# lia2790/walking-controllers

Hardware: AMD Instinct MI355X
Metric: QP solves/sec (whole node), iCub IK-QP + DCM-MPC batch at 1/2/4/8 MI355X (higher is better)
Workload: dtype f64

## Files before the change

walking-controllers_amd/csrc/ik4.hip:

```cpp
#include "ik4_device.h"

namespace {

template <bool TICK, int JSRC, bool LOG = false, bool EXT = false>
__global__ __launch_bounds__(64, WCQP_IK4_WAVES)
void ik4_kernel(const IkDeviceParams* __restrict__ prm, int batch,
                const double* __restrict__ JL, const double* __restrict__ JR,
                const double* __restrict__ JN, const double* __restrict__ JC,
                const double* qpos, const double* __restrict__ state,
                double* __restrict__ dq_out, int* __restrict__ status_out,
                unsigned* __restrict__ alo_out, unsigned* __restrict__ aup_out,
                double* __restrict__ ferr_out, int* __restrict__ iters_out, const wcqp_tick::TickDev* __restrict__ tdp, int phase, int n_inner, int skip_last_mpc)
{
    __shared__ __attribute__((aligned(16))) double smem[4][PER_INST];
    if constexpr (TICK) {
        __shared__ __attribute__((aligned(16))) double kmodel[JSRC == 2 ? wcqp_tick::kKinTabSize : 2];
        __shared__ __attribute__((aligned(16))) double kgains[JSRC == 2 ? 4 * wcqp_tick::kGainsLdsStages : 2];
        ik4_tick_walk<JSRC, LOG, EXT, false>(prm, batch, JL, JR, JN, JC, qpos, state, dq_out, status_out, alo_out, aup_out, ferr_out, iters_out,
                                             tdp, phase, n_inner, skip_last_mpc, smem, kmodel, kgains);
    } else {
        ik4_body<TICK, JSRC>(prm, batch, JL, JR, JN, JC, qpos, state, dq_out, status_out, alo_out, aup_out, ferr_out, iters_out, wcqp_tick::TickDev{}, smem, xcd_group((int)blockIdx.x, (int)gridDim.x));
    }
}

// ... 21 lines not shown
                    unsigned* __restrict__ alo_out, unsigned* __restrict__ aup_out,
                    double* __restrict__ ferr_out, int* __restrict__ iters_out, int ik_blocks, MpcPairArgs m)
{
    __shared__ __attribute__((aligned(16))) double smem[4][PER_INST];
    const bool is_mpc = (int)blockIdx.x >= ik_blocks;
    const int blk = is_mpc ? (int)blockIdx.x - ik_blocks : xcd_group((int)blockIdx.x, ik_blocks);
    if (is_mpc) {
        static_assert(wcqp_mpc::kInstPerWave * WCQP_HULL_ROWS * 4 <= 4 * PER_INST, "the hull rows fit the IK's LDS");
        double (*s_hull)[WCQP_HULL_ROWS][4] = reinterpret_cast<double (*)[WCQP_HULL_ROWS][4]>(&smem[0][0]);
        const int lane = threadIdx.x;
        const int sub = lane / wcqp_mpc::kLanesPerInstance, t = lane % wcqp_mpc::kLanesPerInstance;
        const long inst_raw = (long)blk * wcqp_mpc::kInstPerWave + sub;
        const bool live = inst_raw < batch;
        const long inst = live ? inst_raw : (long)batch - 1;
        const double2* rp = reinterpret_cast<const double2*>(m.ref) + inst * m.ref_len;
        double ux, uy, margin;
        int st;
        unsigned mask;
        wcqp_mpc::mpc_row_solve(m.c, t, inst, m.x0, rp, m.ref_len, m.u_prev, m.hull_A, m.hull_b, m.hull_nc, inst, s_hull[sub], ux, uy, st, mask, margin);
        if (t == 0 && live) {
            reinterpret_cast<double2*>(m.u0)[inst] = make_double2(ux, uy);
            m.status[inst] = st;
            if (m.active) m.active[inst] = mask;
            if (m.margin) m.margin[inst] = margin;
        }
        return;
    }
    ik4_body<false>(prm, batch, JL, JR, JN, JC, qpos, state, dq_out, status_out, alo_out, aup_out, ferr_out, iters_out, wcqp_tick::TickDev{}, smem, blk);
}

template <bool WITH_MPC>
__device__ __forceinline__
void plan_walk(const IkDeviceParams* __restrict__ prm, int batch, const wcqp_qp_step* __restrict__ recs, int n_steps, int ways, int groups,
               const wcqp_mpc::MpcDeviceConsts& c, unsigned* queue, double (*smem)[PER_INST])
{
    const bool dynamic = ways == 0;
    unsigned z = threadIdx.x;
    __asm__ volatile("" : "+v"(z));
    z >>= 6;
    constexpr unsigned QS = wcqp_ik::kPlanQueueStride / 4u;
    const unsigned total = (unsigned)n_steps * (unsigned)groups;
    unsigned home = blockIdx.x % wcqp_ik::kPlanQueues;
    auto draw = [&]() -> unsigned {
#ifndef WCQP_PLAN_STEAL
#define WCQP_PLAN_STEAL (wcqp_ik::kPlanQueues - 1u)
#endif
        for (unsigned tried = 0; tried <= WCQP_PLAN_STEAL; ++tried) {
            unsigned k = 0;
            if (threadIdx.x == 0) k = __hip_atomic_fetch_add(queue + home * QS + z, 1u, __ATOMIC_RELAXED, __HIP_MEMORY_SCOPE_AGENT);
            const unsigned u = (unsigned)__builtin_amdgcn_readfirstlane((int)k) * wcqp_ik::kPlanQueues + home;
            if (u < total) return u;
            home = (home + 1u) % wcqp_ik::kPlanQueues;
        }
        return total;
    };
    int r = (int)blockIdx.x / groups, blk = (int)blockIdx.x % groups;
#ifndef WCQP_PLAN_NO_XCD_MAP
    if ((groups & 7) == 0) {
        const int n = groups >> 3, x = (int)blockIdx.x & 7, k = (int)blockIdx.x >> 3;
        r = k / n; blk = x * n + k % n;
    }
#endif
    if (dynamic) {
        const unsigned u = draw();
        r = u < total ? (int)(u % (unsigned)n_steps) : n_steps; blk = u < total ? (int)(u / (unsigned)n_steps) : 0;
    }
#pragma unroll 1
    while (r < n_steps) {
        __asm__ volatile("" ::: "memory");
        using wcqp::as_global;
        const wcqp_qp_step& s = recs[r];
        MpcPairArgs m{c, WITH_MPC ? as_global(s.x0) : nullptr, WITH_MPC ? as_global(s.ref) : nullptr, s.ref_len, WITH_MPC ? as_global(s.u_prev) : nullptr,
                      WITH_MPC ? as_global(s.hull_A) : nullptr, WITH_MPC ? as_global(s.hull_b) : nullptr, WITH_MPC ? as_global(s.hull_nc) : nullptr,
                      WITH_MPC ? as_global(s.u0) : nullptr, WITH_MPC ? as_global(s.mpc_status) : nullptr, WITH_MPC ? as_global(s.mpc_active) : nullptr,
                      WITH_MPC ? as_global(s.mpc_margin) : nullptr,
                      dynamic ? queue + home * QS + z : nullptr, 0u, WITH_MPC};
        ik4_body<false, 0, true>(prm, batch, as_global(s.J_left), as_global(s.J_right), as_global(s.J_neck), as_global(s.J_com), as_global(s.q), as_global(s.state),
                                 as_global(s.dq), as_global(s.ik_status), as_global(s.active_lower), as_global(s.active_upper),
                                 as_global(s.foot_err), as_global(s.iters), wcqp_tick::TickDev{}, smem, blk, 0, true, nullptr, nullptr, &m);
        wcqp::wave_lds_fence();
        if (dynamic) {
            unsigned u = (unsigned)__builtin_amdgcn_readfirstlane((int)m.ticket) * wcqp_ik::kPlanQueues + home;
            if (u >= total) { home = (home + 1u) % wcqp_ik::kPlanQueues; u = draw(); }
            r = u < total ? (int)(u % (unsigned)n_steps) : n_steps; blk = u < total ? (int)(u / (unsigned)n_steps) : 0;
        } else {
            r += ways;
        }
    }
    if (dynamic && threadIdx.x == 0) {
        __threadfence();
        if (atomicAdd(queue + wcqp_ik::kPlanQueues * QS, 1u) == gridDim.x - 1) {
            for (unsigned q = 0; q <= wcqp_ik::kPlanQueues; ++q) queue[q * QS] = 0u;
        }
    }
}

__global__ __launch_bounds__(64, WCQP_IK4_WAVES)
void qp_plan_kernel(const IkDeviceParams* __restrict__ prm, int batch, const wcqp_qp_step* __restrict__ recs, int n_steps, int ways, int groups,
                    wcqp_mpc::MpcDeviceConsts c, unsigned* queue)
{
    __shared__ __attribute__((aligned(16))) double smem[4][PER_INST];
    plan_walk<true>(prm, batch, recs, n_steps, ways, groups, c, queue, smem);
}
__global__ __launch_bounds__(64, WCQP_IK4_WAVES) WCQP_IK_PLAN_REGS
void ik_plan_kernel(const IkDeviceParams* __restrict__ prm, int batch, const wcqp_qp_step* __restrict__ recs, int n_steps, int ways, int groups,
                    wcqp_mpc::MpcDeviceConsts c, unsigned* queue)
{
    __shared__ __attribute__((aligned(16))) double smem[4][PER_INST];
    plan_walk<false>(prm, batch, recs, n_steps, ways, groups, c, queue, smem);
}

}

namespace wcqp_ik {

int ik4_plan_queue_grid(int batch, int n_steps) {
    int dev = 0, cus = 0;
    if (hipGetDevice(&dev) != hipSuccess || hipDeviceGetAttribute(&cus, hipDeviceAttributeMultiprocessorCount, dev) != hipSuccess || cus < 1) return -1;
    const long long total = (long long)((batch + 3) / 4) * n_steps, slots = (long long)cus * 4 * WCQP_IK4_WAVES;
    return (int)(total < slots ? total : slots);
}

int ik4_launch_plan(const IkDeviceParams* d_prm, int batch, const wcqp_qp_step* d_recs, int n_steps, int ways,
                    const wcqp_mpc::MpcDeviceConsts& c, hipStream_t stream, unsigned* d_queue, int queue_grid, bool ik_only) {
    if (!d_prm || !d_recs || batch < 1 || n_steps < 1 || ways < 0 || (ways == 0 && (!d_queue || queue_grid < 1))) return WCQP_E_INVALID;
    const int groups = (batch + 3) / 4;
    if ((long long)groups * n_steps >= (1ll << 31)) return WCQP_E_INVALID;
    const unsigned grid = ways == 0 ? (unsigned)queue_grid : (unsigned)(groups * ways);
    if (ik_only) hipLaunchKernelGGL(ik_plan_kernel, dim3(grid), dim3(64), 0, stream, d_prm, batch, d_recs, n_steps, ways, groups, c, d_queue);
    else hipLaunchKernelGGL(qp_plan_kernel, dim3(grid), dim3(64), 0, stream, d_prm, batch, d_recs, n_steps, ways, groups, c, d_queue);
    WCQP_HIP_TRY(hipGetLastError());
    return WCQP_OK;
}

int ik4_launch_pair(const IkDeviceParams* d_prm, int batch, const IkIo& io,
                    const wcqp_mpc::MpcDeviceConsts& c, const double* x0, const double* ref, int ref_len, const double* u_prev,
                    const double* hull_A, const double* hull_b, const int* hull_nc,
                    double* u0, int* mstatus, unsigned* mactive, double* mmargin, hipStream_t stream) {
    const int ik_blocks = (batch + 3) / 4;
    const int mpc_blocks = (batch + wcqp_mpc::kInstPerWave - 1) / wcqp_mpc::kInstPerWave;
    MpcPairArgs m{c, x0, ref, ref_len, u_prev, hull_A, hull_b, hull_nc, u0, mstatus, mactive, mmargin};
    hipLaunchKernelGGL(qp_pair_kernel, dim3((unsigned)(ik_blocks + mpc_blocks)), dim3(64), 0, stream, d_prm, batch,
// ... 58 lines not shown
```

walking-controllers_amd/csrc/ik4_device.h:

```cpp
#pragma once
#include <cmath>
#include <limits>
#include <type_traits>
#include "ik_common.h"
#include "tick_device.h"
#include "kin_device.h"

namespace {

using namespace wcqp_ik;

typedef double v4d __attribute__((ext_vector_type(4)));

constexpr int NR = 12;
constexpr int NROWS_IN = 18;
constexpr int KMAX = kDof - 9;
constexpr int LDC = 14;

constexpr int OFF_ST = 0;
constexpr int OFF_BV = 112;
constexpr int OFF_DB = 130;
constexpr int OFF_CT = 0;
constexpr int OFF_PB = 0;
constexpr int A_SIZE = 340;
constexpr int OFF_COL = A_SIZE;
constexpr int OFF_YV = A_SIZE + 32;
constexpr int OFF_DV = A_SIZE + 48;
constexpr int OFF_YPV = A_SIZE;
constexpr int OFF_RV = A_SIZE + 16;
constexpr int OFF_CV = A_SIZE + 32;
constexpr int OFF_ROWB = A_SIZE + 48;
constexpr int PER_INST = 440;
constexpr int K_FS = 14, K_TW = 0, K_FRB = 322, K_FR = 358;
constexpr int K_MS = 394, K_MH = 410;
// ... 29 lines not shown
#elif defined(WCQP_IK_STAMPS)
#define WCQP_STAMP(k) do { unsigned long long t__; asm volatile("s_memtime %0\n\ts_waitcnt lgkmcnt(0)" : "=s"(t__) :: "memory"); \
                           if (lane == __ffsll((long long)__ballot(true)) - 1) reinterpret_cast<unsigned long long*>(ferr_out)[(size_t)blockIdx.x * 16 + (k)] = t__; } while (0)
#else
#define WCQP_STAMP(k) do { } while (0)
#endif
#ifndef WCQP_KSTAMP
#define WCQP_KSTAMP(k) do { } while (0)
#endif

__device__ __forceinline__ void swap32(double& a, double& b) {
    const auto l = __builtin_amdgcn_permlane32_swap((unsigned)__double2loint(a), (unsigned)__double2loint(b), false, false);
    const auto h = __builtin_amdgcn_permlane32_swap((unsigned)__double2hiint(a), (unsigned)__double2hiint(b), false, false);
    a = __hiloint2double((int)h[0], (int)l[0]); b = __hiloint2double((int)h[1], (int)l[1]);
}
__device__ __forceinline__ void swap16(double& a, double& b) {
    const auto l = __builtin_amdgcn_permlane16_swap((unsigned)__double2loint(a), (unsigned)__double2loint(b), false, false);
    const auto h = __builtin_amdgcn_permlane16_swap((unsigned)__double2hiint(a), (unsigned)__double2hiint(b), false, false);
    a = __hiloint2double((int)h[0], (int)l[0]); b = __hiloint2double((int)h[1], (int)l[1]);
}

using wcqp_kin::st2;
using wcqp_kin::ld2;

struct MpcPairArgs {
    wcqp_mpc::MpcDeviceConsts c;
    const double* x0; const double* ref; int ref_len; const double* u_prev;
    const double* hull_A; const double* hull_b; const int* hull_nc;
    double* u0; int* status; unsigned* active; double* margin;
    unsigned* ticket_from = nullptr; unsigned ticket = 0;
    bool has_mpc = true;
};

template <bool TICK, int JSRC = 0, bool PAIR = false, bool LOG = false, bool EXT = false, bool REACT = false, bool GS = false, bool PL = false>
__device__ __forceinline__
void ik4_body(const IkDeviceParams* __restrict__ prm, int batch,
                const double* __restrict__ JL, const double* __restrict__ JR,
                const double* __restrict__ JN, const double* __restrict__ JC,
                const double* qpos, const double* __restrict__ state,
                double* __restrict__ dq_out, int* __restrict__ status_out,
                unsigned* __restrict__ alo_out, unsigned* __restrict__ aup_out,
                double* __restrict__ ferr_out, int* __restrict__ iters_out, const wcqp_tick::TickDev& td, double (*smem)[PER_INST], int blk,
                const int tick_now = 0, const bool do_mpc = true, const double* kmodel = nullptr, const double* gr_lds = nullptr,
                MpcPairArgs* pm = nullptr, double* carry = nullptr, int* gait = nullptr, const unsigned long long* noise_base = nullptr)
{
    static_assert(!(TICK && PAIR), "the tick kernel carries its own MPC chain");
    static_assert(TICK || !REACT, "the reactive controller is a tick form");
    static_assert(TICK || !GS, "gain scheduling is a tick form");
    static_assert(!PL || (TICK && JSRC == 2 && !LOG), "planned / streamed trajectories: the fused-kinematics tick without logger rows");
    constexpr bool ST = PL && EXT;
    constexpr bool COMPACT = JSRC == 1;
    constexpr bool KINF = JSRC == 2;
    int lane_id = threadIdx.x;
    if constexpr (TICK || PAIR) __asm__ volatile("" : "+v"(lane_id));
    const int lane = lane_id;
    const int grp = lane >> 4;
    const int j = lane & 15;
    const long inst_raw = (long)blk * 4 + grp;
    const bool live = inst_raw < batch;
    const long inst = live ? inst_raw : (long)batch - 1;
    using wcqp::at32;
    const unsigned iu = (unsigned)inst, j8 = (unsigned)j * 8u;
    double* S = smem[grp];
    double* st = S + OFF_ST;
    const double inf = std::numeric_limits<double>::infinity();
    const bool var1 = j < kDof - 16;
    const bool rhs1 = j == kDof - 16;
    const bool base1 = j >= 8 && j < 14;
    const int col1 = j + 16;

    unsigned prev_lo = 0u, prev_up = 0u;
    bool stopped = false;
    auto load_previous_set = [&]() {
        if (td.hot_start && alo_out && aup_out) { prev_lo = *at32(alo_out, iu * 4u); prev_up = *at32(aup_out, iu * 4u); }
        stopped = wcqp_tick::tick_robot_stopped(td, (int)inst);
        if (stopped) { prev_lo = 0u; prev_up = 0u; }
    };
    if constexpr (TICK && JSRC != 2) load_previous_set();

    WCQP_STAMP(0);
    const int v0i = 6 + j, v1i = var1 ? 22 + j : 0;
    double sd0, sd1, isd0, isd1, kq0, kq1, qreg0, qreg1;
    auto load_lane_constants = [&]() {
        sd0 = prm->sd[j]; sd1 = prm->sd[col1]; isd0 = prm->isd[j]; isd1 = prm->isd[col1];
        kq0 = prm->kq[v0i]; kq1 = prm->kq[v1i]; qreg0 = prm->qreg[v0i]; qreg1 = prm->qreg[v1i];
    };
    if constexpr (!KINF) load_lane_constants();
    double a0[NROWS_IN], a1[NROWS_IN];
    double q0, q1;
    double qm0, qm1;
    bool osqp_form;
    double k_pos_foot, k_att_foot, k_pos_com, kap;
    int fast_ok;
    wcqp_tick::TickMpcRegs mreg;
    double2 p_xs = make_double2(0.0, 0.0), p_up = make_double2(0.0, 0.0);
    if constexpr (PAIR) {
        if (pm->has_mpc) {
        wcqp_mpc::mpc_window_loads(pm->c, j, reinterpret_cast<const double2*>(pm->ref), iu * (unsigned)pm->ref_len, pm->ref_len, mreg.L);
        if (j == 0) { p_xs = *at32(reinterpret_cast<const double2*>(pm->x0), iu * 16u); p_up = *at32(reinterpret_cast<const double2*>(pm->u_prev), iu * 16u); }
        mreg.nc = *at32(pm->hull_nc, iu * 4u);
        mreg.ha = make_double2(0.0, 0.0); mreg.hb = 0.0;
        if (j < WCQP_HULL_ROWS) {
            mreg.ha = *at32(reinterpret_cast<const double2*>(pm->hull_A), (iu * WCQP_HULL_ROWS + (unsigned)j) * 16u);
            mreg.hb = *at32(pm->hull_b, iu * (WCQP_HULL_ROWS * 8u) + j8);
        }
        }
    }
    if constexpr (TICK && !REACT) { if (do_mpc) wcqp_tick::tick_mpc_issue<KINF>(td, j, inst, tick_now + 1, mreg); else mreg.phase0 = td.phase0[inst]; }
    double2 cr0[5], cr1[5], cdv[5];
    int ckind0 = 0, ckind1 = 0;
    double m_ux = 0.0, m_uy = 0.0;
    double2 m_r0 = make_double2(0.0, 0.0);
    double2 m_rd = make_double2(0.0, 0.0);
    if constexpr (TICK && REACT) { if (do_mpc) wcqp_tick::tick_react_issue(td, j, inst, tick_now + 1, mreg, m_r0, m_rd); else mreg.phase0 = td.phase0[inst]; }
    wcqp_tick::ZmpRegs zreg{};
    double m_s = 0.0;
    auto gsd = [&]() -> const wcqp_tick::TickDevGS& { return static_cast<const wcqp_tick::TickDevGS&>(td); };
    auto pld = [&]() -> const wcqp_tick::TickDevPL& { return static_cast<const wcqp_tick::TickDevPL&>(td); };
    double m_pf = 0.0;
    if constexpr (PL) { if (do_mpc) m_pf = wcqp_tick::plan_flags_issue<ST>(pld(), j, inst, tick_now + 1); }
    if constexpr (TICK && GS) {
        if (do_mpc) {
            wcqp_tick::zmp_state_issue(gsd(), inst, zreg);
            if constexpr (!REACT) m_rd = wcqp_tick::zmp_vel_issue(td, inst, tick_now + 1);
        }
    }
    {
        const unsigned so = iu * (unsigned)(kStateLen * 8);
        const double* sp = at32(state, so + j8);
        const double* sp5 = at32(state, so + 640u + (j < kStateLen - 80 ? j8 : 0u));
// ... 149 lines not shown
                }
                if (!REACT && j < 8) { const double* mh = S + K_MH + j * 3; mreg.ha.x = mh[0]; mreg.ha.y = mh[1]; mreg.hb = mh[2]; }
            }
        } else if constexpr (COMPACT) {
            const double* jb = td.jcomp + inst * td.cstride;
            const int off0 = wcqp_tick::compact_offset(td.cmaskL, td.cmaskR, td.cmaskN, j, ckind0);
            const int off1 = wcqp_tick::compact_offset(td.cmaskL, td.cmaskR, td.cmaskN, var1 ? col1 : 0, ckind1);
#pragma unroll
            for (int m = 0; m < 5; ++m) { cr0[m] = ld2(jb + off0 + 2 * m); cr1[m] = ld2(jb + off1 + 2 * m); }
#pragma unroll
            for (int m = 0; m < 5; ++m) cdv[m] = ld2(jb + td.coff_d + 2 * m);
        } else {
        const int fc0 = 6 + j;
        const int fc1 = var1 ? 22 + j : (base1 ? j - 8 : 0);
        const unsigned o6 = iu * (unsigned)(6 * kNV * 8), o3 = iu * (unsigned)(3 * kNV * 8), c0b = (unsigned)fc0 * 8u, c1b = (unsigned)fc1 * 8u;
        const double* jl0 = at32(JL, o6 + c0b), *jl1 = at32(JL, o6 + c1b);
        const double* jr0 = at32(JR, o6 + c0b), *jr1 = at32(JR, o6 + c1b);
        const double* jc0 = at32(JC, o3 + c0b), *jc1 = at32(JC, o3 + c1b);
        const double* jn0 = at32(JN, o3 + c0b), *jn1 = at32(JN, o3 + c1b);
#pragma unroll
        for (int r = 0; r < 6; ++r) { a0[r] = jl0[r * kNV]; a1[r] = jl1[r * kNV]; }
#pragma unroll
        for (int r = 0; r < 6; ++r) { a0[6 + r] = jr0[r * kNV]; a1[6 + r] = jr1[r * kNV]; }
#pragma unroll
        for (int r = 0; r < 3; ++r) { a0[12 + r] = jc0[r * kNV]; a1[12 + r] = jc1[r * kNV]; }
#pragma unroll
        for (int r = 0; r < 3; ++r) { a0[15 + r] = jn0[r * kNV]; a1[15 + r] = jn1[r * kNV]; }
        }
        __builtin_amdgcn_sched_barrier(0);
        if constexpr (PAIR) {
            if (pm->ticket_from && threadIdx.x == 0) pm->ticket = __hip_atomic_fetch_add(pm->ticket_from, 1u, __ATOMIC_RELAXED, __HIP_MEMORY_SCOPE_AGENT);
            __builtin_amdgcn_sched_barrier(0);
        }
        if constexpr (PAIR) if (pm->has_mpc) {
            double ux, uy, u0x, u0y, margin;
            int mst_;
            unsigned mact;
            wcqp_mpc::mpc_row_partial(pm->c, j, mreg.L, ux, uy);
            if (pm->c.N >= 4 * wcqp_mpc::kLanesPerInstance)
                wcqp_mpc::mpc_row_extra_passes(pm->c, j, reinterpret_cast<const double2*>(pm->ref) + inst * pm->ref_len, pm->ref_len, ux, uy);
            if (j == 0) wcqp_mpc::mpc_row_add_state(pm->c, p_xs, p_up, ux, uy);
            wcqp_mpc::mpc_row_finish(pm->c, j, ux, uy, mreg.nc, mreg.ha.x, mreg.ha.y, mreg.hb, reinterpret_cast<double (*)[4]>(S + OFF_COL), u0x, u0y, mst_, mact, margin);
            if (j == 0 && live) {
                *at32(reinterpret_cast<double2*>(pm->u0), iu * 16u) = make_double2(u0x, u0y);
                *at32(pm->status, iu * 4u) = mst_;
                if (pm->active) *at32(pm->active, iu * 4u) = mact;
                if (pm->margin) *at32(pm->margin, iu * 8u) = margin;
            }
        }
        if constexpr (TICK) {
            double2 kg = make_double2(0.0, 0.0);
            if constexpr (GS) {
                if (do_mpc) {
                    if constexpr (!KINF) m_s = wcqp_tick::zmp_smoother_advance(gsd(), inst, j == 0 && live, m_rd, zreg);
                    kg = wcqp_tick::zmp_gains_at(td, gsd().zg, m_s);
                }
            }
            if constexpr (REACT) {
                if (do_mpc) {
                    if constexpr (!KINF) m_ux = wcqp_tick::tick_react_law(td, j, mreg, m_r0, m_rd);
                    wcqp_tick::tick_react_finish<EXT, GS>(td, j, inst, live, tick_now + 1, mreg, m_r0, m_ux, noise_base, kg);
                }
            } else if (do_mpc) {
                int code1;
                if constexpr (PL) code1 = wcqp_tick::plan_code((int)S[K_PF]);
                else {
                    const int cyc1 = *gait + 1 == 2 * td.step_ticks ? 0 : *gait + 1;
                    code1 = wcqp_tick::contact_code_cyc(cyc1, td.step_ticks, td.ds_ticks);
                }
                if constexpr (KINF) wcqp_tick::tick_mpc_finish_from<false, GS, PL, ST>(td, j, inst, live, tick_now + 1, mreg, m_r0, m_ux, m_uy, reinterpret_cast<double (*)[4]>(S + K_MS), code1, noise_base, kg);
// ... 91 lines not shown
    {
        double acc = q0 + q1 + st[j];
#pragma unroll
        for (int r = 0; r < NROWS_IN; ++r) acc += a0[r] + a1[r];
        if (live) dq_out[inst * kDof + j] = acc + sd0 + sd1 + isd0 + isd1 + kq0 + kq1 + qreg0 + qreg1 + (double)fast_ok + k_pos_foot + k_att_foot + k_pos_com + kap + (osqp_form ? 1.0 : 0.0);
        return;
    }
#endif

    WCQP_STAMP(1);
    double b_mine = 0.0;
    {
        double* bv = S + OFF_BV;
        if (j < 15) {
            if (j < 12) {
                const int foot = j / 6, k = j % 6;
                const double* p  = st + (foot ? 12 : 0);
                const double* R  = st + (foot ? 15 : 3);
                const double* pd = st + (foot ? 36 : 24);
                const double* Rd = st + (foot ? 39 : 27);
                const double* tw = st + (foot ? 81 : 75);
                const double corr = k < 3 ? k_pos_foot * (p[k] - pd[k]) : k_att_foot * rot_err(R, Rd, k - 3);
                const bool skip = osqp_form && tw[0] == tw[1] && tw[0] == 0.0;
                b_mine = skip ? tw[k] : tw[k] - corr;
            } else {
                const int k = j - 12;
                b_mine = st[72 + k] - k_pos_com * (st[66 + k] - st[69 + k]);
            }
            bv[j] = b_mine;
        }
        if (j >= 13) bv[15 + (j - 13)] = kap * rot_err(st + 48, st + 57, j - 13);
    }
    if constexpr (!EXT) { qm0 = q0; qm1 = q1; }
    const double gt0 = -sd0 * kq0 * (qreg0 - qm0);
    const double gt1 = var1 ? -sd1 * kq1 * (qreg1 - qm1) : 0.0;
    wcqp::wave_lds_fence();
    if (rhs1) {
        const double* bv = S + OFF_BV;
#pragma unroll
        for (int r = 0; r < NROWS_IN; r += 2) { const double2 b2 = ld2(bv + r); a1[r] = b2.x; a1[r + 1] = b2.y; }
    }

    WCQP_STAMP(2);
    bool pat = true;
    if constexpr (KINF) {
    } else if constexpr (COMPACT) {
        double* db = S + OFF_DB;
        if (j >= 11 && j < 14) {
            const int cm = j - 11;
            const double e0 = cm == 0 ? 1.0 : 0.0, e1 = cm == 1 ? 1.0 : 0.0, e2 = cm == 2 ? 1.0 : 0.0;
            double Bc[3][3];
#pragma unroll
            for (int f = 0; f < 3; ++f) {
                const double d0 = f == 0 ? cdv[0].x : (f == 1 ? cdv[1].y : cdv[3].x);
                const double d1 = f == 0 ? cdv[0].y : (f == 1 ? cdv[2].x : cdv[3].y);
                const double d2 = f == 0 ? cdv[1].x : (f == 1 ? cdv[2].y : cdv[4].x);
                Bc[f][0] = e1 * d2 - e2 * d1; Bc[f][1] = e2 * d0 - e0 * d2; Bc[f][2] = e0 * d1 - e1 * d0;
            }
#pragma unroll
            for (int r = 0; r < 3; ++r) { db[r * 3 + cm] = Bc[1][r] - Bc[0][r]; db[9 + r * 3 + cm] = Bc[2][r] - Bc[0][r]; }
        }
    } else {
        double* db = S + OFF_DB;
        if (base1) {
            const int cb = j - 8;
            const bool lowc = cb < 3;
// ... 10 lines not shown
            }
            pat = dev <= kMixedTol;
        }
    }
    const bool use = fast_ok != 0 && ((__ballot(!pat) >> (16 * grp)) & 0xffffull) == 0ull;
    wcqp::wave_lds_fence();

    WCQP_STAMP(3);
    double Hr[NR + 1];
    {
        double c0[NR], c1[NR];
        {
            const double* db = S + OFF_DB;
            double dBR[9], dBC[9];
#pragma unroll
            for (int m = 0; m < 8; m += 2) { const double2 v = ld2(db + m); dBR[m] = v.x; dBR[m + 1] = v.y; }
            { const double2 v = ld2(db + 8); dBR[8] = v.x; dBC[0] = v.y; }
#pragma unroll
            for (int m = 1; m < 9; m += 2) { const double2 v = ld2(db + 9 + m); dBC[m] = v.x; dBC[m + 1] = v.y; }
            const double L00 = prm->Lt[0], L01 = prm->Lt[1], L02 = prm->Lt[2], L11 = prm->Lt[4], L12 = prm->Lt[5], L22 = prm->Lt[8];
            auto xf = [&](const double (&a)[NROWS_IN], double sc, double (&c)[NR]) {
                const double w0 = a[3], w1 = a[4], w2 = a[5];
                const double n0 = a[15] - w0, n1 = a[16] - w1, n2 = a[17] - w2;
                c[0] = sc * (L00 * n0 + L01 * n1 + L02 * n2);
                c[1] = sc * (L11 * n1 + L12 * n2);
                c[2] = sc * (L22 * n2);
#pragma unroll
                for (int r = 0; r < 3; ++r) {
                    c[3 + r] = sc * (a[6 + r] - a[r] - (dBR[3 * r] * w0 + dBR[3 * r + 1] * w1 + dBR[3 * r + 2] * w2));
                    c[9 + r] = sc * (a[12 + r] - a[r] - (dBC[3 * r] * w0 + dBC[3 * r + 1] * w1 + dBC[3 * r + 2] * w2));
                }
                c[6] = sc * (a[9] - w0); c[7] = sc * (a[10] - w1); c[8] = sc * (a[11] - w2);
            };
            xf(a0, sd0, c0);
            xf(a1, var1 ? sd1 : 1.0, c1);
        }
        wcqp::wave_lds_fence();
        WCQP_STAMP(4);
        double* ct = S + OFF_CT;
        double* dv = S + OFF_DV;
        {
            double* c = ct + j * LDC;
#pragma unroll
            for (int r = 0; r < NR; r += 2) st2(c + r, c0[r], c0[r + 1]);
            st2(c + NR, gt0, 0.0);
        }
        if (j < 8) {
            double* c = ct + col1 * LDC;
#pragma unroll
            for (int r = 0; r < NR; r += 2) st2(c + r, rhs1 ? 0.0 : c1[r], rhs1 ? 0.0 : c1[r + 1]);
            st2(c + NR, gt1, 0.0);
        }
        if (rhs1) {
#pragma unroll
            for (int r = 0; r < NR; r += 2) st2(dv + r, c1[r], c1[r + 1]);
            ct[24 * LDC] = 0.0; ct[24 * LDC + 1] = 0.0;
        }
    }
    wcqp::wave_lds_fence();
    WCQP_STAMP(10);
    {
        const int mk = lane & 15, mq = lane >> 4;
        v4d acc[4];
#pragma unroll
        for (int g = 0; g < 4; ++g) acc[g] = v4d{0.0, 0.0, 0.0, 0.0};
#pragma unroll
// ... 3 lines not shown
                const double v = smem[g][OFF_CT + (4 * s + mq) * LDC + mk];
                acc[g] = __builtin_amdgcn_mfma_f64_16x16x4f64(v, v, acc[g], 0, 0, 0);
            }
        }
        WCQP_STAMP(11);
        double t[4][4];
#pragma unroll
        for (int reg = 0; reg < 4; ++reg) {
            double x0 = acc[0][reg], x1 = acc[1][reg], x2 = acc[2][reg], x3 = acc[3][reg];
            swap32(x0, x2); swap32(x1, x3);
            swap16(x0, x1); swap16(x2, x3);
            t[0][reg] = x0; t[1][reg] = x1; t[2][reg] = x2; t[3][reg] = x3;
        }
        const double* dv = S + OFF_DV;
        const bool rowok = j < NR, is12 = j == NR;
        const double dj = dv[j < NR ? j : 0];
        const double sgn = rowok ? 1.0 : (is12 ? -1.0 : 0.0), m12 = is12 ? 1.0 : 0.0, mrow = rowok ? -1.0 : 0.0;
#pragma unroll
        for (int k = 0; k < NR; k += 2) {
            const double2 d2 = ld2(dv + k);
            const double h0 = t[k & 3][k >> 2], h1 = t[(k + 1) & 3][(k + 1) >> 2];
            double v0 = fma(m12, d2.x, h0), v1 = fma(m12, d2.y, h1);
            if (k < 3) v0 += (k == j) ? 1.0 : 0.0;
            if (k + 1 < 3) v1 += (k + 1 == j) ? 1.0 : 0.0;
            Hr[k] = sgn * v0;
            Hr[k + 1] = sgn * v1;
        }
        Hr[NR] = mrow * (t[NR & 3][NR >> 2] + dj);
    }

    WCQP_STAMP(5);
    const double tol = prm->tol;
    const int max_iter = prm->max_iter;
    double lo0 = prm->vlo[v0i] * isd0, hi0 = prm->vhi[v0i] * isd0, lo1 = prm->vlo[v1i] * isd1, hi1 = prm->vhi[v1i] * isd1;
    bool ok = true;
    {
        double* col = S + OFF_COL;
        static_assert(OFF_DV + 16 == OFF_COL + 64, "the column pairs take the 64 doubles of region B");
        double pmin = 1.0;
        col[j] = Hr[0];
        col[16 + j] = Hr[1];
        wcqp::wave_lds_fence();
#pragma unroll
        for (int k = 0; k < NR; k += 2) {
            const int buf = (k >> 1) & 1;
            const double* cA = col + 32 * buf;
            const double* cB = cA + 16;
            double ca[NR + 2], cb2[NR + 2];
#pragma unroll
            for (int q = 0; q <= NR; q += 2) {
                const double2 x2 = ld2(cA + q), y2 = ld2(cB + q);
                ca[q] = x2.x; ca[q + 1] = x2.y; cb2[q] = y2.x; cb2[q + 1] = y2.y;
            }
            const double pa = ca[k], pb = ca[k + 1], pd = cb2[k + 1];
            const double det = fma(pa, pd, -pb * pb);
            pmin = (pa > 0.0 && det > 0.0) ? pmin : -1.0;
            const double idet = wcqp::fast_rcp(det);
            const double i11 = pd * idet, i12 = -pb * idet, i22 = pa * idet;
            const double m1 = Hr[k], m2 = Hr[k + 1];
            const double g1 = fma(m1, i11, m2 * i12), g2 = fma(m1, i12, m2 * i22);
            const double ek = (j == k) ? 1.0 : 0.0, ek1 = (j == k + 1) ? 1.0 : 0.0;
            const double f1 = fma(-ek1, i12, fma(-ek, i11, g1));
            const double f2 = fma(-ek1, i22, fma(-ek, i12, g2));
            if (k + 2 < NR) {
                Hr[k + 2] = fma(-f2, cb2[k + 2], fma(-f1, ca[k + 2], Hr[k + 2]));
                Hr[k + 3] = fma(-f2, cb2[k + 3], fma(-f1, ca[k + 3], Hr[k + 3]));
                double* nb = col + 32 * (buf ^ 1);
// ... 463 lines not shown
                            wcqp::wave_lds_fence();
                            const int wdrop = Wi(jd);
                            double myjd = 0.0;
                            const double djj = rowb[jd];
                            myjd = rowb[j < KMAX ? j : 0];
                            const double f = (s_live && j != jd) ? myjd * wcqp::fast_rcp(djj) : 0.0;
#pragma unroll
                            for (int b = 0; b < KMAX; b += 2) {
                                const double2 d2 = ld2(rowb + b);
                                myR[b] = (j == jd || b == jd) ? 0.0 : fma(-f, d2.x, myR[b]);
                                myR[b + 1] = (j == jd || b + 1 == jd) ? 0.0 : fma(-f, d2.y, myR[b + 1]);
                            }
                            if (j == jd) { s_live = false; s_mu = 0.0; }
                            if (wdrop == j) { in_w0 = false; sig0 = 0.0; }
                            if (wdrop == col1) { in_w1 = false; sig1 = 0.0; }
                            --nW;
                            ++it;
                        }
                    }
                }
                wcqp::wave_lds_fence();
            }
        }
        {
            const double d0 = in_w0 ? fabs(nu0 - (sig0 > 0.0 ? hi0 : lo0)) : fmax(nu0 - hi0, lo0 - nu0);
            const double d1 = !bnd1 ? 0.0 : (in_w1 ? fabs(nu1 - (sig1 > 0.0 ? hi1 : lo1)) : fmax(nu1 - hi1, lo1 - nu1));
            const double dev = fmax(d0 == d0 ? d0 : inf, d1 == d1 ? d1 : inf);
            const unsigned bad = row_max_u32((dev > 1e-9) ? 1u : 0u);
            if (st_code == WCQP_STATUS_SOLVED && bad != 0u) st_code = WCQP_STATUS_NUMERIC;
        }
    }

    WCQP_STAMP(8);
    double dq0 = nu0 * sd0, dq1 = nu1 * sd1;
    if (st_code == WCQP_STATUS_SOLVED && in_w0) dq0 = sig0 > 0.0 ? prm->vhi[v0i] : prm->vlo[v0i];
    if (st_code == WCQP_STATUS_SOLVED && in_w1) dq1 = sig1 > 0.0 ? prm->vhi[v1i] : prm->vlo[v1i];
    const bool nonfinite = row_max_u32((isfinite(dq0) && (!var1 || isfinite(dq1))) ? 0u : 1u) != 0u;
    if (nonfinite) { st_code = WCQP_STATUS_NUMERIC; dq0 = 0.0; dq1 = 0.0; in_w0 = false; in_w1 = false; }
    const unsigned long long bu0 = __ballot(in_w0 && sig0 > 0.0), bu1 = __ballot(in_w1 && sig1 > 0.0);
    const unsigned long long bl0 = __ballot(in_w0 && sig0 < 0.0), bl1 = __ballot(in_w1 && sig1 < 0.0);
    if (!use) {
        st_code = WCQP_STATUS_STRUCTURE;
        dq0 = 0.0; dq1 = 0.0;
    }
    if (live) {
        double* dqo = at32(dq_out, iu * (unsigned)(kDof * 8) + j8);
        dqo[0] = dq0;
        if (var1) dqo[16] = dq1;
        if (j == 0) {
            const unsigned up = (unsigned)((bu0 >> (16 * grp)) & 0xffffull) | ((unsigned)((bu1 >> (16 * grp)) & 0x7full) << 16);
            const unsigned dn = (unsigned)((bl0 >> (16 * grp)) & 0xffffull) | ((unsigned)((bl1 >> (16 * grp)) & 0x7full) << 16);
            *at32(status_out, iu * 4u) = st_code;
            if (aup_out) *at32(aup_out, iu * 4u) = use ? up : 0u;
            if (alo_out) *at32(alo_out, iu * 4u) = use ? dn : 0u;
            if (iters_out) *at32(iters_out, iu * 4u) = it;
        }
    }
#ifdef WCQP_IK_STAMPS
    WCQP_STAMP(9);
    return;
#endif
    if constexpr (TICK) {
        const bool ik_ok = st_code == WCQP_STATUS_SOLVED;
        if (live) {
            const int i_ = (int)inst;
            const double v0 = (ik_ok && !stopped) ? dq0 : 0.0, v1 = (ik_ok && !stopped) ? dq1 : 0.0;
            carry[0] += 0.5 * td.dT * (v0 + carry[2]); carry[2] = v0;
            const size_t g0 = (size_t)i_ * kDof + j;
            double* qd = at32(td.q_des.get(), iu * (unsigned)(kDof * 8) + j8), *dp = at32(td.dq_prev.get(), iu * (unsigned)(kDof * 8) + j8);
// ... 165 lines not shown
```

walking-controllers_amd/csrc/mpc.hip:

```cpp
#include <cmath>
#include <cstring>
#include <limits>
#include <new>
#include "wcqp_internal.h"
#include "mpc_device.h"

namespace {

using namespace wcqp_mpc;
constexpr int kBlock = 64;

__global__ __launch_bounds__(kBlock)
void mpc_condensed_kernel(MpcDeviceConsts c, int batch,
                          const double* __restrict__ x0, const double* __restrict__ ref, int ref_len,
                          int ref_stride, const int* __restrict__ ref_start,
                          const double* __restrict__ u_prev,
                          const double* __restrict__ hull_A, const double* __restrict__ hull_b,
                          const int* __restrict__ hull_nc, int hull_sets, const int* __restrict__ hull_sel,
                          double* __restrict__ u0_out, int* __restrict__ status_out,
                          unsigned* __restrict__ active_out, double* __restrict__ margin_out)
{
    __shared__ __attribute__((aligned(16))) double s_hull[kInstPerWave][WCQP_HULL_ROWS][4];

    const int lane = threadIdx.x;
    const int sub  = lane / kLanesPerInstance;
    const int t    = lane % kLanesPerInstance;
    const long inst_raw = (long)blockIdx.x * kInstPerWave + sub;
    const bool live = inst_raw < batch;
    const long inst = live ? inst_raw : (long)batch - 1;

    const int start = ref_start ? *ref_start : 0;
    const double2* rp = reinterpret_cast<const double2*>(ref) + inst * ref_stride + start;
    const long hset = inst * hull_sets + (hull_sel ? hull_sel[inst] : 0);
    double ux, uy, margin;
    int st;
    unsigned mask;
    mpc_row_solve(c, t, inst, x0, rp, ref_len, u_prev, hull_A, hull_b, hull_nc, hset, s_hull[sub], ux, uy, st, mask, margin);
    if (t == 0 && live) {
        reinterpret_cast<double2*>(u0_out)[inst] = make_double2(ux, uy);
        status_out[inst] = st;
        if (active_out) active_out[inst] = mask;
        if (margin_out) margin_out[inst] = margin;
    }
}

#ifdef WCQP_MPC_PLAN_VGPR_HALF
__attribute__((amdgpu_num_vgpr(WCQP_MPC_PLAN_VGPR_HALF)))
#endif
__global__ __launch_bounds__(kBlock)
void mpc_plan_kernel(MpcDeviceConsts c, int batch, const wcqp_qp_step* __restrict__ recs, int n_steps, int ways, int groups)
{
    __shared__ __attribute__((aligned(16))) double s_hull[kInstPerWave][WCQP_HULL_ROWS][4];
    using wcqp::as_global;
    const int way = (int)blockIdx.x / groups, blk = (int)blockIdx.x % groups;
#pragma unroll 1
    for (int r = way; r < n_steps; r += ways) {
        __asm__ volatile("" ::: "memory");
        int lane = threadIdx.x;
        __asm__ volatile("" : "+v"(lane));
        const int sub = lane / kLanesPerInstance, t = lane % kLanesPerInstance;
        const long inst_raw = (long)blk * kInstPerWave + sub;
        const bool live = inst_raw < batch;
        const long inst = live ? inst_raw : (long)batch - 1;
        const wcqp_qp_step& s = recs[r];
        const double2* rp = reinterpret_cast<const double2*>(as_global(s.ref)) + inst * s.ref_len;
        double ux, uy, margin;
        int st;
        unsigned mask;
        mpc_row_solve(c, t, inst, as_global(s.x0), rp, s.ref_len, as_global(s.u_prev), as_global(s.hull_A), as_global(s.hull_b), as_global(s.hull_nc), inst,
                      s_hull[sub], ux, uy, st, mask, margin);
        if (t == 0 && live) {
            reinterpret_cast<double2*>(as_global(s.u0))[inst] = make_double2(ux, uy);
            as_global(s.mpc_status)[inst] = st;
            if (s.mpc_active) as_global(s.mpc_active)[inst] = mask;
            if (s.mpc_margin) as_global(s.mpc_margin)[inst] = margin;
        }
        wcqp::wave_lds_fence();
    }
}

}

struct wcqp_mpc_s {
    wcqp_mpc_params p{};
    int N = 0, n = 0, nx = 0, nu = 0;
    double a = 0, b = 0;
    std::vector<double> P, Aeq, grad_sub;
    std::vector<double> Gr;
    double Gx[4]{}, Gu[4]{}, S0[4]{};
    double* d_Gr = nullptr;
    int device = -1;
    wcqp::DeviceScratch scratch;
};

namespace {

void matmul_tn(const std::vector<double>& A, const std::vector<double>& B, std::vector<double>& C,
               int k, int r, int c) {
    C.assign((size_t)r * c, 0.0);
    for (int kk = 0; kk < k; ++kk)
        for (int i = 0; i < r; ++i) {
            const double aik = A[(size_t)kk * r + i];
            if (aik == 0.0) continue;
// ... 231 lines not shown
```

walking-controllers_amd/csrc/mpc_device.h:

```cpp
#pragma once
#include <limits>
#include "wcqp_internal.h"
#include "gptr.h"

namespace wcqp_mpc {

constexpr int kLanesPerInstance = 16;
constexpr int kInstPerWave = 64 / kLanesPerInstance;

struct MpcDeviceConsts {
    wcqp::GPtr<const double> Gr;
    double Gx[4], Gu[4], S0[4];
    double feas_tol, hull_tol;
    int N;
};

#if defined(__HIPCC__)
__device__ __forceinline__ int pair_e(int k) { return (int)(((k < 16 ? 0x2221111110000000ull : 0x655444333322ull) >> (4 * (k & 15))) & 7ull); }
__device__ __forceinline__ int pair_f(int k) { return (int)(((k < 16 ? 0x5437654327654321ull : 0x776765765476ull) >> (4 * (k & 15))) & 7ull); }
constexpr int kNumCand = 1 + 8 + 28;

template <int CTRL>
__device__ __forceinline__ double row_move(double v) {
    const int lo = wcqp::dpp_dword<CTRL>(__double2loint(v));
    const int hi = wcqp::dpp_dword<CTRL>(__double2hiint(v));
    return __hiloint2double(hi, lo);
}
template <int CTRL>
__device__ __forceinline__ int row_move(int v) { return wcqp::dpp_dword<CTRL>(v); }
#define WCQP_ROW_STEPS(X) X(0xB1) X(0x4E) X(0x141) X(0x140)

struct MpcLoads {
    double2 r[4], g0[4], g1[4];
};
__device__ __forceinline__ void mpc_window_loads(const MpcDeviceConsts& c, int t, const double2* __restrict__ ref, unsigned w0, int ref_len, MpcLoads& L)
{
    const double2* gp = reinterpret_cast<const double2*>(c.Gr.get());
#pragma unroll
    for (int k = 0; k < 4; ++k) {
        const int i = t + k * kLanesPerInstance;
        const int ic = i <= c.N ? i : c.N;
// ... 200 lines not shown
```

Baseline: 1.205 billion.

## Stage IK lane constants and MPC gain table in LDS for plan kernels

```diff
diff --git a/walking-controllers_amd/csrc/ik4.hip b/walking-controllers_amd/csrc/ik4.hip
--- a/walking-controllers_amd/csrc/ik4.hip
+++ b/walking-controllers_amd/csrc/ik4.hip
@@ -77,8 +77,9 @@
 template <bool WITH_MPC>
 __device__ __forceinline__
 void plan_walk(const IkDeviceParams* __restrict__ prm, int batch, const wcqp_qp_step* __restrict__ recs, int n_steps, int ways, int groups,
-               const wcqp_mpc::MpcDeviceConsts& c, unsigned* queue, double (*smem)[PER_INST])
-{
+               const wcqp_mpc::MpcDeviceConsts& c, unsigned* queue, double (*smem)[PER_INST], double* ptab)
+{
+    constexpr int TAB = WITH_MPC ? WCQP_PLAN_LDS : (WCQP_PLAN_LDS & 2);
     const bool dynamic = ways == 0;
     unsigned z = threadIdx.x;
     __asm__ volatile("" : "+v"(z));
@@ -106,6 +107,8 @@
         r = k / n; blk = x * n + k % n;
     }
 #endif
+    PlanTables pt;
+    plan_tables_issue<TAB>(prm, c, WITH_MPC, ptab, pt);
     if (dynamic) {
         const unsigned u = draw();
         r = u < total ? (int)(u % (unsigned)n_steps) : n_steps; blk = u < total ? (int)(u / (unsigned)n_steps) : 0;
@@ -120,10 +123,11 @@
                       WITH_MPC ? as_global(s.u0) : nullptr, WITH_MPC ? as_global(s.mpc_status) : nullptr, WITH_MPC ? as_global(s.mpc_active) : nullptr,
                       WITH_MPC ? as_global(s.mpc_margin) : nullptr,
                       dynamic ? queue + home * QS + z : nullptr, 0u, WITH_MPC};
-        ik4_body<false, 0, true>(prm, batch, as_global(s.J_left), as_global(s.J_right), as_global(s.J_neck), as_global(s.J_com), as_global(s.q), as_global(s.state),
+        ik4_body<false, 0, true, false, false, false, false, false, TAB>(prm, batch, as_global(s.J_left), as_global(s.J_right), as_global(s.J_neck), as_global(s.J_com), as_global(s.q), as_global(s.state),
                                  as_global(s.dq), as_global(s.ik_status), as_global(s.active_lower), as_global(s.active_upper),
-                                 as_global(s.foot_err), as_global(s.iters), wcqp_tick::TickDev{}, smem, blk, 0, true, nullptr, nullptr, &m);
+                                 as_global(s.foot_err), as_global(s.iters), wcqp_tick::TickDev{}, smem, blk, 0, true, nullptr, nullptr, &m, nullptr, nullptr, nullptr, &pt);
         wcqp::wave_lds_fence();
+        pt.fill = false; pt.f_ik[0] = pt.f_ik[1] = pt.f_ik[2] = 0.0; pt.f_gr[0] = pt.f_gr[1] = make_double2(0.0, 0.0);
         if (dynamic) {
             unsigned u = (unsigned)__builtin_amdgcn_readfirstlane((int)m.ticket) * wcqp_ik::kPlanQueues + home;
             if (u >= total) { home = (home + 1u) % wcqp_ik::kPlanQueues; u = draw(); }
@@ -145,14 +149,16 @@
                     wcqp_mpc::MpcDeviceConsts c, unsigned* queue)
 {
     __shared__ __attribute__((aligned(16))) double smem[4][PER_INST];
-    plan_walk<true>(prm, batch, recs, n_steps, ways, groups, c, queue, smem);
+    __shared__ __attribute__((aligned(16))) double ptab[PT_SIZE];
+    plan_walk<true>(prm, batch, recs, n_steps, ways, groups, c, queue, smem, ptab);
 }
 __global__ __launch_bounds__(64, WCQP_IK4_WAVES) WCQP_IK_PLAN_REGS
 void ik_plan_kernel(const IkDeviceParams* __restrict__ prm, int batch, const wcqp_qp_step* __restrict__ recs, int n_steps, int ways, int groups,
                     wcqp_mpc::MpcDeviceConsts c, unsigned* queue)
 {
     __shared__ __attribute__((aligned(16))) double smem[4][PER_INST];
-    plan_walk<false>(prm, batch, recs, n_steps, ways, groups, c, queue, smem);
+    __shared__ __attribute__((aligned(16))) double ptab[PT_GR];
+    plan_walk<false>(prm, batch, recs, n_steps, ways, groups, c, queue, smem, ptab);
 }
 
 }
diff --git a/walking-controllers_amd/csrc/ik4_device.h b/walking-controllers_amd/csrc/ik4_device.h
--- a/walking-controllers_amd/csrc/ik4_device.h
+++ b/walking-controllers_amd/csrc/ik4_device.h
@@ -1,5 +1,6 @@
 #pragma once
 #include <cmath>
+#include <cstddef>
 #include <limits>
 #include <type_traits>
 #include "ik_common.h"
@@ -95,7 +96,58 @@
     bool has_mpc = true;
 };
 
-template <bool TICK, int JSRC = 0, bool PAIR = false, bool LOG = false, bool EXT = false, bool REACT = false, bool GS = false, bool PL = false>
+#ifndef WCQP_PLAN_LDS
+#define WCQP_PLAN_LDS 3
+#endif
+constexpr int kPlanGrStages = wcqp_mpc::kGrLdsStages;
+constexpr int PT_KQ = 0, PT_QREG = 32, PT_VLO = 64, PT_VHI = 96, PT_SD = 128, PT_ISD = 160;
+constexpr int PT_GR = 192;
+constexpr int PT_SIZE = PT_GR + 4 * kPlanGrStages;
+static_assert(offsetof(IkDeviceParams, qreg) == offsetof(IkDeviceParams, kq) + 256 && offsetof(IkDeviceParams, vlo) == offsetof(IkDeviceParams, kq) + 512 &&
+              offsetof(IkDeviceParams, vhi) == offsetof(IkDeviceParams, kq) + 768 && offsetof(IkDeviceParams, isd) == offsetof(IkDeviceParams, sd) + 256,
+              "kq | qreg | vlo | vhi and sd | isd are copied as two runs");
+static_assert(PT_GR % 2 == 0 && (4 * PER_INST + PT_SIZE) * 8 <= 20480, "eight plan workgroups per CU: two waves per SIMD");
+struct PlanTables {
+    double* lds;
+    bool gr_staged;
+    bool fill;
+    double f_ik[3];
+    double2 f_gr[2];
+};
+template <int TAB>
+__device__ __forceinline__ void plan_tables_issue(const IkDeviceParams* prm, const wcqp_mpc::MpcDeviceConsts& c, bool with_mpc, double* lds, PlanTables& pt)
+{
+    const unsigned l8 = threadIdx.x * 8u;
+    pt.lds = lds; pt.fill = true;
+    pt.f_ik[0] = pt.f_ik[1] = pt.f_ik[2] = 0.0;
+    pt.f_gr[0] = pt.f_gr[1] = make_double2(0.0, 0.0);
+    if constexpr ((TAB & 2) != 0) {
+        const double* t4 = reinterpret_cast<const double*>(reinterpret_cast<const char*>(prm) + offsetof(IkDeviceParams, kq));
+        const double* t2 = reinterpret_cast<const double*>(reinterpret_cast<const char*>(prm) + offsetof(IkDeviceParams, sd));
+        pt.f_ik[0] = *wcqp::at32(t4, l8); pt.f_ik[1] = *wcqp::at32(t4, l8 + 512u); pt.f_ik[2] = *wcqp::at32(t2, l8);
+    }
+    pt.gr_staged = false;
+    if constexpr ((TAB & 1) != 0) {
+        pt.gr_staged = with_mpc && c.N < kPlanGrStages;
+        if (pt.gr_staged) {
+            const double2* gp = reinterpret_cast<const double2*>(c.Gr.get());
+            const unsigned last = 2u * (unsigned)c.N + 1u, e0 = threadIdx.x, e1 = threadIdx.x + 64u;
+            pt.f_gr[0] = *wcqp::at32(gp, (e0 < last ? e0 : last) * 16u); pt.f_gr[1] = *wcqp::at32(gp, (e1 < last ? e1 : last) * 16u);
+        }
+    }
+}
+template <int TAB>
+__device__ __forceinline__ void plan_tables_land(const PlanTables& pt, int lane)
+{
+    double* T = pt.lds;
+    if constexpr ((TAB & 2) != 0) { T[lane] = pt.f_ik[0]; T[64 + lane] = pt.f_ik[1]; T[PT_SD + lane] = pt.f_ik[2]; }
+    if constexpr ((TAB & 1) != 0) {
+        if (pt.gr_staged) { st2(T + PT_GR + 2 * lane, pt.f_gr[0].x, pt.f_gr[0].y); st2(T + PT_GR + 128 + 2 * lane, pt.f_gr[1].x, pt.f_gr[1].y); }
+    }
+    wcqp::wave_lds_fence();
+}
+
+template <bool TICK, int JSRC = 0, bool PAIR = false, bool LOG = false, bool EXT = false, bool REACT = false, bool GS = false, bool PL = false, int TAB = 0>
 __device__ __forceinline__
 void ik4_body(const IkDeviceParams* __restrict__ prm, int batch,
                 const double* __restrict__ JL, const double* __restrict__ JR,
@@ -105,9 +157,14 @@
                 unsigned* __restrict__ alo_out, unsigned* __restrict__ aup_out,
                 double* __restrict__ ferr_out, int* __restrict__ iters_out, const wcqp_tick::TickDev& td, double (*smem)[PER_INST], int blk,
                 const int tick_now = 0, const bool do_mpc = true, const double* kmodel = nullptr, const double* gr_lds = nullptr,
-                MpcPairArgs* pm = nullptr, double* carry = nullptr, int* gait = nullptr, const unsigned long long* noise_base = nullptr)
+                MpcPairArgs* pm = nullptr, double* carry = nullptr, int* gait = nullptr, const unsigned long long* noise_base = nullptr,
+                const PlanTables* pt = nullptr)
 {
     static_assert(!(TICK && PAIR), "the tick kernel carries its own MPC chain");
+    static_assert(TAB == 0 || (PAIR && JSRC == 0), "the LDS tables are the plan kernels'");
+    constexpr bool TAB_GR = (TAB & 1) != 0, TAB_IK = (TAB & 2) != 0;
+    const double* ptab = nullptr;
+    if constexpr (TAB != 0) ptab = pt->lds;
     static_assert(TICK || !REACT, "the reactive controller is a tick form");
     static_assert(TICK || !GS, "gain scheduling is a tick form");
     static_assert(!PL || (TICK && JSRC == 2 && !LOG), "planned / streamed trajectories: the fused-kinematics tick without logger rows");
@@ -148,7 +205,7 @@
         sd0 = prm->sd[j]; sd1 = prm->sd[col1]; isd0 = prm->isd[j]; isd1 = prm->isd[col1];
         kq0 = prm->kq[v0i]; kq1 = prm->kq[v1i]; qreg0 = prm->qreg[v0i]; qreg1 = prm->qreg[v1i];
     };
-    if constexpr (!KINF) load_lane_constants();
+    if constexpr (!KINF && !TAB_IK) load_lane_constants();
     double a0[NROWS_IN], a1[NROWS_IN];
     double q0, q1;
     double qm0, qm1;
@@ -159,6 +216,10 @@
     double2 p_xs = make_double2(0.0, 0.0), p_up = make_double2(0.0, 0.0);
     if constexpr (PAIR) {
         if (pm->has_mpc) {
+        if constexpr (TAB_GR) {
+            if (pt->gr_staged) wcqp_mpc::mpc_window_loads_ref_only(pm->c, j, reinterpret_cast<const double2*>(pm->ref), iu * (unsigned)pm->ref_len, pm->ref_len, mreg.L);
+            else wcqp_mpc::mpc_window_loads(pm->c, j, reinterpret_cast<const double2*>(pm->ref), iu * (unsigned)pm->ref_len, pm->ref_len, mreg.L);
+        } else
         wcqp_mpc::mpc_window_loads(pm->c, j, reinterpret_cast<const double2*>(pm->ref), iu * (unsigned)pm->ref_len, pm->ref_len, mreg.L);
         if (j == 0) { p_xs = *at32(reinterpret_cast<const double2*>(pm->x0), iu * 16u); p_up = *at32(reinterpret_cast<const double2*>(pm->u_prev), iu * 16u); }
         mreg.nc = *at32(pm->hull_nc, iu * 4u);
@@ -374,10 +435,17 @@
             if (pm->ticket_from && threadIdx.x == 0) pm->ticket = __hip_atomic_fetch_add(pm->ticket_from, 1u, __ATOMIC_RELAXED, __HIP_MEMORY_SCOPE_AGENT);
             __builtin_amdgcn_sched_barrier(0);
         }
+        if constexpr (TAB != 0) {
+            if (pt->fill) plan_tables_land<TAB>(*pt, lane);
+        }
         if constexpr (PAIR) if (pm->has_mpc) {
             double ux, uy, u0x, u0y, margin;
             int mst_;
             unsigned mact;
+            if constexpr (TAB_GR) {
+                if (pt->gr_staged) wcqp_mpc::mpc_row_partial_lds(pm->c, j, mreg.L, ptab + PT_GR, ux, uy);
+                else wcqp_mpc::mpc_row_partial(pm->c, j, mreg.L, ux, uy);
+            } else
             wcqp_mpc::mpc_row_partial(pm->c, j, mreg.L, ux, uy);
             if (pm->c.N >= 4 * wcqp_mpc::kLanesPerInstance)
                 wcqp_mpc::mpc_row_extra_passes(pm->c, j, reinterpret_cast<const double2*>(pm->ref) + inst * pm->ref_len, pm->ref_len, ux, uy);
@@ -535,6 +603,10 @@
         if (j >= 13) bv[15 + (j - 13)] = kap * rot_err(st + 48, st + 57, j - 13);
     }
     if constexpr (!EXT) { qm0 = q0; qm1 = q1; }
+    if constexpr (TAB_IK) {
+        sd0 = ptab[PT_SD + j]; sd1 = ptab[PT_SD + col1]; kq0 = ptab[PT_KQ + v0i]; kq1 = ptab[PT_KQ + v1i];
+        qreg0 = ptab[PT_QREG + v0i]; qreg1 = ptab[PT_QREG + v1i];
+    }
     const double gt0 = -sd0 * kq0 * (qreg0 - qm0);
     const double gt1 = var1 ? -sd1 * kq1 * (qreg1 - qm1) : 0.0;
     wcqp::wave_lds_fence();
@@ -611,6 +683,7 @@
                 }
                 c[6] = sc * (a[9] - w0); c[7] = sc * (a[10] - w1); c[8] = sc * (a[11] - w2);
             };
+            if constexpr (TAB_IK) { sd0 = ptab[PT_SD + j]; sd1 = ptab[PT_SD + col1]; }
             xf(a0, sd0, c0);
             xf(a1, var1 ? sd1 : 1.0, c1);
         }
@@ -680,7 +753,13 @@
     WCQP_STAMP(5);
     const double tol = prm->tol;
     const int max_iter = prm->max_iter;
-    double lo0 = prm->vlo[v0i] * isd0, hi0 = prm->vhi[v0i] * isd0, lo1 = prm->vlo[v1i] * isd1, hi1 = prm->vhi[v1i] * isd1;
+    double lo0, hi0, lo1, hi1;
+    if constexpr (TAB_IK) {
+        isd0 = ptab[PT_ISD + j]; isd1 = ptab[PT_ISD + col1];
+        lo0 = ptab[PT_VLO + v0i] * isd0; hi0 = ptab[PT_VHI + v0i] * isd0; lo1 = ptab[PT_VLO + v1i] * isd1; hi1 = ptab[PT_VHI + v1i] * isd1;
+    } else {
+        lo0 = prm->vlo[v0i] * isd0; hi0 = prm->vhi[v0i] * isd0; lo1 = prm->vlo[v1i] * isd1; hi1 = prm->vhi[v1i] * isd1;
+    }
     bool ok = true;
     {
         double* col = S + OFF_COL;
@@ -1210,9 +1289,16 @@
     }
 
     WCQP_STAMP(8);
+    if constexpr (TAB_IK) { sd0 = ptab[PT_SD + j]; sd1 = ptab[PT_SD + col1]; }
     double dq0 = nu0 * sd0, dq1 = nu1 * sd1;
+    if constexpr (TAB_IK) {
+        const double bl0 = ptab[PT_VLO + v0i], bh0 = ptab[PT_VHI + v0i], bl1 = ptab[PT_VLO + v1i], bh1 = ptab[PT_VHI + v1i];
+        if (st_code == WCQP_STATUS_SOLVED && in_w0) dq0 = sig0 > 0.0 ? bh0 : bl0;
+        if (st_code == WCQP_STATUS_SOLVED && in_w1) dq1 = sig1 > 0.0 ? bh1 : bl1;
+    } else {
     if (st_code == WCQP_STATUS_SOLVED && in_w0) dq0 = sig0 > 0.0 ? prm->vhi[v0i] : prm->vlo[v0i];
     if (st_code == WCQP_STATUS_SOLVED && in_w1) dq1 = sig1 > 0.0 ? prm->vhi[v1i] : prm->vlo[v1i];
+    }
     const bool nonfinite = row_max_u32((isfinite(dq0) && (!var1 || isfinite(dq1))) ? 0u : 1u) != 0u;
     if (nonfinite) { st_code = WCQP_STATUS_NUMERIC; dq0 = 0.0; dq1 = 0.0; in_w0 = false; in_w1 = false; }
     const unsigned long long bu0 = __ballot(in_w0 && sig0 > 0.0), bu1 = __ballot(in_w1 && sig1 > 0.0);
diff --git a/walking-controllers_amd/csrc/mpc.hip b/walking-controllers_amd/csrc/mpc.hip
--- a/walking-controllers_amd/csrc/mpc.hip
+++ b/walking-controllers_amd/csrc/mpc.hip
@@ -47,12 +47,22 @@
 #ifdef WCQP_MPC_PLAN_VGPR_HALF
 __attribute__((amdgpu_num_vgpr(WCQP_MPC_PLAN_VGPR_HALF)))
 #endif
-__global__ __launch_bounds__(kBlock)
+__global__ __launch_bounds__(kBlock, 6)
 void mpc_plan_kernel(MpcDeviceConsts c, int batch, const wcqp_qp_step* __restrict__ recs, int n_steps, int ways, int groups)
 {
     __shared__ __attribute__((aligned(16))) double s_hull[kInstPerWave][WCQP_HULL_ROWS][4];
+    __shared__ __attribute__((aligned(16))) double s_gr[4 * kGrLdsStages];
     using wcqp::as_global;
     const int way = (int)blockIdx.x / groups, blk = (int)blockIdx.x % groups;
+    const bool staged = c.N < kGrLdsStages;
+    if (staged) {
+        const double2* gp = reinterpret_cast<const double2*>(c.Gr.get());
+        const unsigned last = 2u * (unsigned)c.N + 1u, e0 = threadIdx.x, e1 = threadIdx.x + 64u;
+        const double2 f0 = gp[e0 < last ? e0 : last], f1 = gp[e1 < last ? e1 : last];
+        double* g = s_gr + 2 * threadIdx.x;
+        g[0] = f0.x; g[1] = f0.y; g[128] = f1.x; g[129] = f1.y;
+        wcqp::wave_lds_fence();
+    }
 #pragma unroll 1
     for (int r = way; r < n_steps; r += ways) {
         __asm__ volatile("" ::: "memory");
@@ -67,8 +77,30 @@
         double ux, uy, margin;
         int st;
         unsigned mask;
-        mpc_row_solve(c, t, inst, as_global(s.x0), rp, s.ref_len, as_global(s.u_prev), as_global(s.hull_A), as_global(s.hull_b), as_global(s.hull_nc), inst,
-                      s_hull[sub], ux, uy, st, mask, margin);
+        if (staged) {
+            MpcLoads L;
+#pragma unroll
+            for (int k = 0; k < 4; ++k) {
+                const int i = t + k * kLanesPerInstance;
+                const int ic = i <= c.N ? i : c.N;
+                L.r[k] = rp[ic < s.ref_len ? ic : s.ref_len - 1];
+            }
+            double2 xs = make_double2(0.0, 0.0), up = xs, ha = xs;
+            double hb = 0.0;
+            if (t == 0) { xs = reinterpret_cast<const double2*>(as_global(s.x0))[inst]; up = reinterpret_cast<const double2*>(as_global(s.u_prev))[inst]; }
+            const int nc = as_global(s.hull_nc)[inst];
+            if (t < WCQP_HULL_ROWS) {
+                ha = reinterpret_cast<const double2*>(as_global(s.hull_A))[inst * WCQP_HULL_ROWS + t];
+                hb = as_global(s.hull_b)[inst * WCQP_HULL_ROWS + t];
+            }
+            double px, py;
+            mpc_row_partial_lds(c, t, L, s_gr, px, py);
+            if (t == 0) mpc_row_add_state(c, xs, up, px, py);
+            mpc_row_finish(c, t, px, py, nc, ha.x, ha.y, hb, s_hull[sub], ux, uy, st, mask, margin);
+        } else {
+            mpc_row_solve(c, t, inst, as_global(s.x0), rp, s.ref_len, as_global(s.u_prev), as_global(s.hull_A), as_global(s.hull_b), as_global(s.hull_nc), inst,
+                          s_hull[sub], ux, uy, st, mask, margin);
+        }
         if (t == 0 && live) {
             reinterpret_cast<double2*>(as_global(s.u0))[inst] = make_double2(ux, uy);
             as_global(s.mpc_status)[inst] = st;
diff --git a/walking-controllers_amd/csrc/mpc_device.h b/walking-controllers_amd/csrc/mpc_device.h
--- a/walking-controllers_amd/csrc/mpc_device.h
+++ b/walking-controllers_amd/csrc/mpc_device.h
@@ -7,6 +7,7 @@
 
 constexpr int kLanesPerInstance = 16;
 constexpr int kInstPerWave = 64 / kLanesPerInstance;
+constexpr int kGrLdsStages = 4 * kLanesPerInstance;
 
 struct MpcDeviceConsts {
     wcqp::GPtr<const double> Gr;
```

Result: faster. 1.225 billion (median of 6 runs) (+1.7%).
